# johncai117/Meta-Fine-Tuning

Measured on AMD Instinct MI355X. Metric: episodes/sec at 5-way N-shot (ResNet10+GNN) per GPU and 1/2/4/8-GPU node, higher is better.
Workload: dtype f32

## Files before the change

meta-fine-tuning_amd/csrc/conv_igemm.hip:

```cpp
#include "mft_common.h"
#include "mft_hip_testing.h"

int mft_stem_conv_dispatch(const float* in, const float* w, float* out, int n_img, int H, int W, int w_ld,
                           hipStream_t s);
int mft_skinny_fwd_dispatch(const float* in, int ldi, const float* w, float* out, int ldo, int n_img, int H, int W,
                            int Cin, int Cout, int KH, int KW, int stride, int pad, int imgs_per_group,
                            long long w_group_stride, hipStream_t s);
void mft_skinny_set_dgrad_slices(int n);
void mft_skinny_set_tap(int v);
void mft_skinny_set_x3(int v);
void mft_skinny_set_nw(int v);
void mft_bn_small_set_rows(int rows);
void mft_bn_fwd_small_set_rows(int rows);
void mft_skinny_set_lines(int v);
int mft_skinny_dgrad_dispatch(const float* dy, int ldy, const float* w, float* dx, int ldx, int n_img, int H, int W,
                              int Cin, int Cout, int KH, int KW, int stride, int pad, int imgs_per_group,
                              long long w_group_stride, hipStream_t s);

namespace {

struct ConvArgs {
    const float* in;
    const float* w;
    const float* bias;
    float* out;
    int ldi, ldo;
    int H, W, Cin, OH, OW, Cout, KH, KW, stride, pad;
    int Kpad;
    int Ktot;
    int rows_per_group;
    int imgs_per_group;
    int tiles_n;
    long long wgs;
    int bt_stride;
    int ksplit;
    float* ws;
    int parity;
};

constexpr int BK = 32;
constexpr int LDS_LD = 36;
int g_dgrad_parity = 1;
int g_wgrad_tile = 64;
int g_conv_tile = 0;
int g_wgrad_pol = 7;
int g_wgrad_trim = 1;
int g_wgrad_rows = 1;
int g_wgrad_early = 1;
int g_wgrad_min_lds_kb = 0;
int g_skinny = 1;
int g_stem_fast = 1;

template <int BM, int BN, int WM, int WN, bool STEM, bool BT>
__global__ __launch_bounds__(256) void conv_igemm_kernel(ConvArgs p) {
    constexpr int TM = BM / WM / 32;
    constexpr int TN = BN / WN / 32;
    constexpr int PA = BM / 32;
    constexpr int PB = BN / 32;
    extern __shared__ __attribute__((aligned(16))) float smem[];

    const int tid = threadIdx.x;
    const int lane = tid & 63;
    const int wave = tid >> 6;
    const int wm = wave / WN, wn = wave % WN;
    const int r = lane & 31, h = lane >> 5;

    int tile_id = blockIdx.x;
    if (gridDim.y == 1) {
        const int nwg = gridDim.x, q = nwg >> 3, rmd = nwg & 7;
        const int xcd = tile_id & 7, slot = tile_id >> 3;
        tile_id = xcd * q + (xcd < rmd ? xcd : rmd) + slot;
    }
    const int nt = tile_id % p.tiles_n;
    const int mt = tile_id / p.tiles_n;
    const bool par = BT && p.parity != 0;
    const int g = par ? 0 : blockIdx.y;
    const int ph = par ? (int)(blockIdx.y >> 1) : 0, pw = par ? (int)(blockIdx.y & 1) : 0;
    const int Hc = par ? (p.OH - ph + 1) / 2 : p.OH, Wc = par ? (p.OW - pw + 1) / 2 : p.OW;
    const int rows = par ? p.imgs_per_group * Hc * Wc : p.rows_per_group;
    const int m0 = mt * BM, n0 = nt * BN;
    if (par && m0 >= rows) return;
    const int kh0 = par ? ((ph - p.pad) & 1) : 0, kw0 = par ? ((pw - p.pad) & 1) : 0;
    const int nkh = par ? (p.KH - kh0 + 1) / 2 : p.KH, nkw = par ? (p.KW - kw0 + 1) / 2 : p.KW;

    const int lrow = tid >> 3;
    const int c4 = (tid & 7) * 4;
    const int ohw = Hc * Wc;

    long long a_base[PA];
    int a_ih0[PA], a_iw0[PA];
    bool a_ok[PA];
#pragma unroll
    for (int j = 0; j < PA; ++j) {
        int m = m0 + lrow + 32 * j;
        a_ok[j] = m < rows;
        int mm = a_ok[j] ? m : 0;
        int img = mm / ohw;
// ... 1041 lines not shown
    a.wgs = (groups > 1) ? w_group_stride : 0;
    a.tiles_n = 0;
    a.bt_stride = 1;
    a.ksplit = 1; a.ws = nullptr; a.parity = 0;
    if (ws != nullptr && !stem && ldo % 4 == 0) {
        a.ksplit = conv_ksplit(a.rows_per_group, Cout, a.Kpad, groups);
        a.ws = ws;
    }
    hipStream_t s = (hipStream_t)stream;
    if (stem) {
        if (g_stem_fast && KH == 7 && KW == 7 && stride == 2 && pad == 3 && Cout == 64 && ldi == 3 && ldo == 64 &&
            bias == nullptr && (W == 84 || W == 224)) {
            const int rc = mft_stem_conv_dispatch(in, w, out, n_img, H, W, a.Kpad, s);
            if (rc != MFT_EINVAL) return rc;
        }
        return launch_conv<128, 64, 2, 2, true>(a, groups, s);
    }
    if (g_skinny && groups > 1 && w_group_stride != 0 && bias == nullptr && ws == nullptr) {
        const int rc = mft_skinny_fwd_dispatch(in, ldi, w, out, ldo, n_img, H, W, Cin, Cout, KH, KW, stride, pad,
                                               imgs_per_group, w_group_stride, s);
        if (rc != MFT_EINVAL) return rc;
    }
    int tile = g_conv_tile;
    if (tile == 0) tile = (Cout >= 64) ? 4 : 5;
    switch (tile) {
        case 1: return launch_conv<128, 128, 2, 2, false>(a, groups, s);
        case 2: return launch_conv<128, 64, 2, 2, false>(a, groups, s);
        case 3: return launch_conv<64, 128, 2, 2, false>(a, groups, s);
        case 4: return launch_conv<64, 64, 2, 2, false>(a, groups, s);
        default: return launch_conv<128, 32, 4, 1, false>(a, groups, s);
    }
}

extern "C" int mft_conv2d_nhwc(const float* in, int ldi, const float* w, const float* bias, float* out, int ldo,
                               int n_img, int H, int W, int Cin, int Cout, int KH, int KW, int stride, int pad,
                               int imgs_per_group, long long w_group_stride, void* stream) {
    return conv2d_impl(in, ldi, w, bias, out, ldo, n_img, H, W, Cin, Cout, KH, KW, stride, pad, imgs_per_group, w_group_stride,
                       nullptr, stream);
}

extern "C" long long mft_conv_ksplit_ws_floats(long long rows, int cols, int K) {
    const int s = conv_ksplit(rows, cols, K);
    return s > 1 ? (long long)s * rows * cols : 0;
}

extern "C" long long mft_conv_ksplit_grouped_ws_floats(long long rows_per_group, int cols, int K, int groups) {
    const int s = conv_ksplit(rows_per_group, cols, K, groups);
    return s > 1 ? (long long)s * groups * rows_per_group * cols : 0;
}

extern "C" int mft_conv2d_nhwc_ksplit_grouped(const float* in, int ldi, const float* w, float* out, int ldo, int n_img, int H, int W,
                                              int Cin, int Cout, int KH, int KW, int stride, int pad, int imgs_per_group,
                                              long long w_group_stride, float* ws, void* stream) {
    if (ws == nullptr || imgs_per_group <= 0) return MFT_EINVAL;
    return conv2d_impl(in, ldi, w, nullptr, out, ldo, n_img, H, W, Cin, Cout, KH, KW, stride, pad, imgs_per_group, w_group_stride, ws,
                       stream);
}

extern "C" int mft_conv2d_nhwc_ksplit(const float* in, int ldi, const float* w, const float* bias, float* out, int ldo,
                                      int n_img, int H, int W, int Cin, int Cout, int KH, int KW, int stride, int pad, float* ws,
                                      void* stream) {
    return conv2d_impl(in, ldi, w, bias, out, ldo, n_img, H, W, Cin, Cout, KH, KW, stride, pad, 0, 0, ws, stream);
}

extern "C" int mft_has_experiments(void) {
#ifdef MFT_EXPERIMENTS
    return 1;
#else
    return 0;
#endif
}

extern "C" int mft_debug_set_conv_tile(int tile) {
#ifndef MFT_EXPERIMENTS
    if (tile == 9502 || tile == 9504 || tile == 9505) return MFT_EINVAL;
    if (tile >= 9000 && tile < 9100 && tile != 9003 && tile != 9007) return MFT_EINVAL;
    if (tile > 4000 && tile < 5000) return MFT_EINVAL;
#endif
    if (tile >= 11000) { mft_bn_small_set_rows(tile - 11000); mft_bn_fwd_small_set_rows(tile - 11000); }
    else if (tile >= 9800) g_dgrad_parity = tile - 9800;
    else if (tile >= 9700) mft_skinny_set_lines(tile - 9700);
    else if (tile >= 9600) g_wgrad_trim = tile - 9600;
    else if (tile >= 9500) g_wgrad_rows = tile - 9500;
    else if (tile >= 9100) mft_skinny_set_nw(tile - 9100);
    else if (tile >= 9000) g_wgrad_pol = tile - 9000;
    else if (tile >= 8000) mft_skinny_set_x3(tile - 8000);
    else if (tile >= 7000) mft_skinny_set_tap(tile - 7000);
    else if (tile >= 6000) mft_skinny_set_dgrad_slices(tile - 6000);
    else if (tile >= 5000) g_wgrad_early = tile - 5000;
    else if (tile >= 4000) g_wgrad_min_lds_kb = tile - 4000;
    else if (tile >= 3000) g_skinny = tile - 3000;
    else if (tile >= 2100) g_stem_wgrad_strips = tile - 2100;
    else if (tile >= 2000) g_stem_fast = tile - 2000;
    else if (tile >= 1000) g_wgrad_tile = tile - 1000;
    else g_conv_tile = tile;
    return 0;
}

extern "C" int mft_debug_set_x3_tile(int t);

extern "C" void mft_wgrad_fwd_set_exact(int on);
extern "C" int mft_debug_reset(void) {
    mft_wgrad_fwd_set_exact(0);
    mft_wgrad_fwd_set_xcd(1);
    g_dgrad_parity = 1; g_wgrad_trim = 1; g_wgrad_rows = 1; g_wgrad_tile = 64; g_conv_tile = 0; g_wgrad_pol = 7; g_wgrad_early = 1; g_wgrad_min_lds_kb = 0; g_skinny = 1; g_stem_fast = 1; g_stem_wgrad_strips = 1;
    mft_skinny_set_lines(1); mft_skinny_set_nw(0); mft_skinny_set_x3(1); mft_skinny_set_tap(1); mft_skinny_set_dgrad_slices(1);
    mft_debug_set_x3_tile(0); mft_debug_set_x3_tile(10); mft_debug_set_x3_tile(21); mft_debug_set_x3_tile(31); mft_debug_set_x3_tile(41);
    mft_bn_small_set_rows(512); mft_bn_fwd_small_set_rows(512);
    mft_debug_set_x3_tile(60); mft_debug_set_x3_tile(70); mft_debug_set_x3_tile(80); mft_debug_set_x3_tile(91); mft_debug_set_x3_tile(100); mft_debug_set_x3_tile(200);
    return 0;
}

static int dgrad_impl(const float* dy, int ldy, const float* w, float* dx, int ldx, int n_img, int H,
                      int W, int Cin, int Cout, int KH, int KW, int stride, int pad,
                      int imgs_per_group, long long w_group_stride, float* ws, void* stream) {
    if (Cout % 32 != 0 || Cin % 4 != 0 || ldy % 4 != 0 || stride < 1) return MFT_EINVAL;
    if (imgs_per_group <= 0) imgs_per_group = n_img;
    if (n_img % imgs_per_group != 0) return MFT_EINVAL;
    const int groups = n_img / imgs_per_group;
    if (g_skinny && groups > 1 && w_group_stride != 0 && ws == nullptr) {
        const int rc = mft_skinny_dgrad_dispatch(dy, ldy, w, dx, ldx, n_img, H, W, Cin, Cout, KH, KW, stride, pad,
                                                 imgs_per_group, w_group_stride, (hipStream_t)stream);
        if (rc != MFT_EINVAL) return rc;
    }
    ConvArgs a;
    a.in = dy; a.w = w; a.bias = nullptr; a.out = dx;
    a.ldi = ldy; a.ldo = ldx;
    a.H = (H + 2 * pad - KH) / stride + 1;
    a.W = (W + 2 * pad - KW) / stride + 1;
    a.Cin = Cout; a.KH = KH; a.KW = KW;
    a.stride = 1; a.pad = -pad;
    a.bt_stride = stride;
    a.OH = H; a.OW = W;
    a.Cout = Cin;
    a.Ktot = KH * KW * Cout;
    a.Kpad = a.Ktot;
    a.imgs_per_group = imgs_per_group;
    a.rows_per_group = imgs_per_group * H * W;
    a.wgs = (groups > 1) ? w_group_stride : 0;
    a.tiles_n = 0;
    a.ksplit = 1; a.ws = nullptr;
    a.parity = (groups == 1 && stride == 2 && g_dgrad_parity) ? 1 : 0;
    if (ws != nullptr && ldx % 4 == 0 && Cin % 64 == 0) {
        const int s_full = conv_ksplit(a.rows_per_group, Cin, a.Kpad, groups);
        if (!a.parity) {
            a.ksplit = s_full;
            a.ws = ws;
        } else if (s_full > 1) {
            int sp = conv_ksplit((long long)imgs_per_group * ((H + 1) / 2) * ((W + 1) / 2), Cin, ((KH + 1) / 2) * ((KW + 1) / 2) * Cout, 4);
            if (sp > s_full) sp = s_full;
            if (sp > 1) { a.ksplit = sp; a.ws = ws; }
        }
    }
    hipStream_t s = (hipStream_t)stream;
    if (Cin % 64 == 0) return launch_conv<64, 64, 2, 2, false, true>(a, groups, s);
    return launch_conv<128, 32, 4, 1, false, true>(a, groups, s);
}

extern "C" int mft_conv2d_dgrad_nhwc(const float* dy, int ldy, const float* w, float* dx, int ldx, int n_img, int H,
                                     int W, int Cin, int Cout, int KH, int KW, int stride, int pad,
                                     int imgs_per_group, long long w_group_stride, void* stream) {
    return dgrad_impl(dy, ldy, w, dx, ldx, n_img, H, W, Cin, Cout, KH, KW, stride, pad, imgs_per_group, w_group_stride, nullptr,
                      stream);
}

extern "C" int mft_conv2d_dgrad_nhwc_ksplit_grouped(const float* dy, int ldy, const float* w, float* dx, int ldx, int n_img, int H,
                                                    int W, int Cin, int Cout, int KH, int KW, int stride, int pad, int imgs_per_group,
                                                    long long w_group_stride, float* ws, void* stream) {
    if (ws == nullptr || imgs_per_group <= 0 || stride != 1) return MFT_EINVAL;
    return dgrad_impl(dy, ldy, w, dx, ldx, n_img, H, W, Cin, Cout, KH, KW, stride, pad, imgs_per_group, w_group_stride, ws, stream);
}

extern "C" int mft_conv2d_dgrad_nhwc_ksplit(const float* dy, int ldy, const float* w, float* dx, int ldx, int n_img, int H, int W,
                                            int Cin, int Cout, int KH, int KW, int stride, int pad, float* ws, void* stream) {
    return dgrad_impl(dy, ldy, w, dx, ldx, n_img, H, W, Cin, Cout, KH, KW, stride, pad, 0, 0, ws, stream);
}

extern "C" long long mft_conv2d_wgrad_ws_floats(int n_img, int H, int W, int Cin, int Cout, int KH, int KW, int stride,
                                                 int pad, int imgs_per_group) {
    if (imgs_per_group <= 0) imgs_per_group = n_img;
    const int OH = (H + 2 * pad - KH) / stride + 1, OW = (W + 2 * pad - KW) / stride + 1;
    const long long rows = (long long)imgs_per_group * OH * OW;
    int chunk_rows, chunks;
    wgrad_chunking(rows, wgrad_wgs_per_chunk(Cin, Cout, KH, KW, n_img / imgs_per_group), &chunk_rows, &chunks);
    if (chunks <= 1) return 0;
    const long long kpad = (KH * KW * Cin + 31) / 32 * 32;
    return (long long)(n_img / imgs_per_group) * chunks * Cout * kpad;
}

// ... 122 lines not shown
```

meta-fine-tuning_amd/csrc/skinny.hip:

```cpp
#include "mft_common.h"

namespace {

typedef float f32x4v __attribute__((ext_vector_type(4)));

struct SkinnyArgs {
    const float* act;
    const float* w;
    float* out;
    int lda, ldo;
    int H, W, Cin, OH, OW, Cout, KH, KW, stride, pad;
    int ipg, rows_in, rows_out;
    long long wgs;
    int K;
    int CS;
};

constexpr int SK_PADF = 8;
constexpr int SK_U = 8;

__global__ __launch_bounds__(1024) void skinny_conv_fwd_kernel(SkinnyArgs p) {
    extern __shared__ __attribute__((aligned(16))) float lds[];
    const int tid = threadIdx.x;
    const int lane = tid & 63, wave = tid >> 6;
// ... 718 lines not shown
    auto wptr = [&](int qq) { return qq < n_groups ? sk_wptr<LN>(wrow, qq, p.K) : sk_wptr<LN>(wsrow, qq - n_groups, p.Cin); };
    f32x4v a_cur[SK_U];
#pragma unroll
    for (int u = 0; u < SK_U; ++u) a_cur[u] = __builtin_nontemporal_load((const f32x4v*)sk_wptr<LN>(wrow, u, p.K));
    gather(0);
    scatter(0);
    __syncthreads();
    auto pass_body = [&](int pass, f32x4v (&A)[3]) {
        const unsigned short* L = ldh + (pass & 1) * 3 * PL + 8 * kq;
        for (int cg0 = 0; cg0 < gpt; cg0 += SK_U) {
            const int q0 = pass * gpt + cg0;
            const bool more = q0 + SK_U < n_groups + gpt;
#pragma unroll
            for (int u = 0; u < SK_U; u += 2) {
                bf16x8 a[3], b[3][3];
                sk_wfix<LN>(a_cur[u], a_cur[u + 1]);
                sk_split_a(a_cur[u], a_cur[u + 1], a);
                if (more) {
                    a_cur[u] = __builtin_nontemporal_load((const f32x4v*)wptr(q0 + SK_U + u));
                    a_cur[u + 1] = __builtin_nontemporal_load((const f32x4v*)wptr(q0 + SK_U + u + 1));
                }
#pragma unroll
                for (int nb = 0; nb < 3; ++nb)
#pragma unroll
                    for (int pl = 0; pl < 3; ++pl)
                        b[nb][pl] = __builtin_bit_cast(bf16x8, *(const u32x4v*)(L + pl * PL + (nb * 16 + m) * RS + (cg0 + u) * 16));
                SK_X3_MFMA(A, a, b)
            }
        }
    };
    for (int pass = 0; pass < taps; ++pass) {
        gather(pass + 1);
        pass_body(pass, acc);
        scatter((pass + 1) & 1);
        __syncthreads();
    }
    pass_body(taps, acs);

    const float inv = 1.f / (float)p.rows_out;
    f32x4v s = {0.f, 0.f, 0.f, 0.f};
#pragma unroll
    for (int nb = 0; nb < 3; ++nb)
        if (nb * 16 + m < p.rows_out) s += acc[nb];
    f32x4v mu, rs;
#pragma unroll
    for (int e = 0; e < 4; ++e) mu[e] = sk_row16_sum(s[e]) * inv;
    s = f32x4v{0.f, 0.f, 0.f, 0.f};
#pragma unroll
    for (int nb = 0; nb < 3; ++nb)
        if (nb * 16 + m < p.rows_out) {
            const f32x4v d = acc[nb] - mu;
            s += d * d;
        }
#pragma unroll
    for (int e = 0; e < 4; ++e) rs[e] = 1.0f / sqrtf(sk_row16_sum(s[e]) * inv + q.eps);
    const int co = co0 + 4 * kq;
    const f32x4v ga = *(const f32x4v*)(q.gamma + g * q.gbs + co), be = *(const f32x4v*)(q.beta + g * q.gbs + co);
    if (m == 0) {
        *(f32x4v*)(q.mean + (long long)g * p.Cout + co) = mu;
        *(f32x4v*)(q.rstd + (long long)g * p.Cout + co) = rs;
    }
    const long long ob = (long long)g * p.rows_out * p.ldo;
#pragma unroll
    for (int nb = 0; nb < 3; ++nb) {
        const int ro = nb * 16 + m;
        if (ro >= p.rows_out) continue;
        const long long o = ob + (long long)ro * p.ldo + co;
        *(f32x4v*)(p.out + o) = acc[nb];
        *(f32x4v*)(q.sc + o) = acs[nb];
        f32x4v y = (acc[nb] - mu) * rs * ga + be;
#pragma unroll
        for (int e = 0; e < 4; ++e) y[e] = fmaxf(y[e], 0.f);
        *(f32x4v*)(q.r1 + o) = y;
    }
}

struct SkinnyBnArgs {
    const float* x_raw;
    const float* relu_out;
    const float* mean; const float* rstd; const float* gamma; long long gbs;
    float* dgamma; float* dbeta;
};

template <bool BNB, int NW>
__global__ __launch_bounds__(64 * NW) void skinny_conv_dgrad_x3_kernel(SkinnyArgs p, SkinnyBnArgs bn) {
    extern __shared__ __attribute__((aligned(16))) unsigned short ldh[];
    typedef float f32x2v __attribute__((ext_vector_type(2)));
    const int tid = threadIdx.x;
    const int lane = tid & 63, wave = tid >> 6;
    const int m = lane & 15, kq = lane >> 4;
    const int g = blockIdx.y;
    const int ci0 = blockIdx.x * (32 * NW) + wave * 32;
    const int Cdy = p.Cin, Cdx = p.Cout;
    const int RS = Cdy + SK_PADH;
    const int PL = p.rows_in * RS;
    const int hw = p.H * p.W;
    const int taps = p.KH * p.KW;
    const long long co_stride = (long long)taps * Cdx;

    int n_img[3], n_h[3], n_w[3];
    bool n_ok[3];
#pragma unroll
    for (int nb = 0; nb < 3; ++nb) {
        const int ro = nb * 16 + m;
        n_ok[nb] = ro < p.rows_out;
        const int rr = n_ok[nb] ? ro : 0;
        const int img = rr / hw;
        const int rem = rr - img * hw;
        n_img[nb] = img;
        n_h[nb] = rem / p.W;
        n_w[nb] = rem - n_h[nb] * p.W;
    }
    const float* wbase = p.w + (long long)g * p.wgs + ci0 + 2 * m;
    const float* actg = p.act + (long long)g * p.rows_in * p.lda;

    constexpr int U = 4;
    const int gpt = Cdy / 16;
    const int n_groups = taps * gpt;
    f32x2v a_cur[U][4];
    auto load_group = [&](int q, f32x2v* dst) {
        const int tap = q / gpt;
        const int cg = q - tap * gpt;
#pragma unroll
        for (int t = 0; t < 4; ++t) {
            const int co = cg * 16 + 4 * kq + t;
            dst[t] = __builtin_nontemporal_load((const f32x2v*)(wbase + (long long)co * co_stride + (long long)tap * Cdx));
        }
    };
#pragma unroll
    for (int u = 0; u < U; ++u) load_group(u, a_cur[u]);
    {
        const int q4 = Cdy / 4;
        for (int i = tid; i < p.rows_in * q4; i += 64 * NW) {
            const int r = i / q4, c = (i - r * q4) * 4;
            sk_store3(ldh, r * RS + sk_perm(c), PL, *(const f32x4v*)(actg + (long long)r * p.lda + c));
        }
    }
    __syncthreads();

    f32x4v acc[2][3];
#pragma unroll
    for (int b = 0; b < 2; ++b)
#pragma unroll
        for (int nb = 0; nb < 3; ++nb) acc[b][nb] = f32x4v{0.f, 0.f, 0.f, 0.f};

    for (int q0 = 0; q0 < n_groups; q0 += U) {
        const bool more = q0 + U < n_groups;
        const int tap = q0 / gpt;
        const int cg0 = q0 - tap * gpt;
        const int kh = tap / p.KW, kw = tap - kh * p.KW;
        int boff[3];
#pragma unroll
        for (int nb = 0; nb < 3; ++nb) {
            const int ih = n_h[nb] + p.pad - kh, iw = n_w[nb] + p.pad - kw;
            const bool ok = n_ok[nb] && ih >= 0 && ih < p.H && iw >= 0 && iw < p.W;
            boff[nb] = ok ? ((n_img[nb] * p.H + ih) * p.W + iw) * RS + 8 * kq + cg0 * 16 : -1;
        }
#pragma unroll
        for (int u = 0; u < U; u += 2) {
            bf16x8 a[2][3], b[3][3];
#pragma unroll
            for (int bb = 0; bb < 2; ++bb) {
                const f32x4v w0 = {a_cur[u][0][bb], a_cur[u][1][bb], a_cur[u][2][bb], a_cur[u][3][bb]};
                const f32x4v w1 = {a_cur[u + 1][0][bb], a_cur[u + 1][1][bb], a_cur[u + 1][2][bb], a_cur[u + 1][3][bb]};
                sk_split_a(w0, w1, a[bb]);
            }
            if (more) {
                load_group(q0 + U + u, a_cur[u]);
                load_group(q0 + U + u + 1, a_cur[u + 1]);
            }
#pragma unroll
            for (int nb = 0; nb < 3; ++nb)
#pragma unroll
                for (int pl = 0; pl < 3; ++pl) {
                    u32x4v z = {0u, 0u, 0u, 0u};
                    if (boff[nb] >= 0) z = *(const u32x4v*)(ldh + pl * PL + boff[nb] + u * 16);
                    b[nb][pl] = __builtin_bit_cast(bf16x8, z);
                }
            SK_X3_MFMA(acc[0], a[0], b)
            SK_X3_MFMA(acc[1], a[1], b)
        }
    }
    float* outg = p.out + (long long)g * p.rows_out * p.ldo;
    f32x4v d[3][2];
#pragma unroll
    for (int nb = 0; nb < 3; ++nb) {
        d[nb][0][0] = acc[0][nb][0]; d[nb][0][1] = acc[1][nb][0]; d[nb][0][2] = acc[0][nb][1]; d[nb][0][3] = acc[1][nb][1];
        d[nb][1][0] = acc[0][nb][2]; d[nb][1][1] = acc[1][nb][2]; d[nb][1][2] = acc[0][nb][3]; d[nb][1][3] = acc[1][nb][3];
    }
    const int cc = ci0 + 8 * kq;
    if constexpr (BNB) {
        const long long gb = (long long)g * p.rows_out * p.ldo;
        f32x4v mu[2], rs[2], ga[2], xh[3][2], s1[2], s2[2];
#pragma unroll
        for (int h = 0; h < 2; ++h) {
            mu[h] = *(const f32x4v*)(bn.mean + (long long)g * Cdx + cc + 4 * h);
            rs[h] = *(const f32x4v*)(bn.rstd + (long long)g * Cdx + cc + 4 * h);
            ga[h] = *(const f32x4v*)(bn.gamma + g * bn.gbs + cc + 4 * h);
            s1[h] = s2[h] = f32x4v{0.f, 0.f, 0.f, 0.f};
        }
#pragma unroll
        for (int nb = 0; nb < 3; ++nb) {
            const int ro = nb * 16 + m;
#pragma unroll
            for (int h = 0; h < 2; ++h) {
                xh[nb][h] = f32x4v{0.f, 0.f, 0.f, 0.f};
                if (ro < p.rows_out) {
                    const long long o = gb + (long long)ro * p.ldo + cc + 4 * h;
                    const f32x4v r = *(const f32x4v*)(bn.relu_out + o);
                    xh[nb][h] = (*(const f32x4v*)(bn.x_raw + o) - mu[h]) * rs[h];
#pragma unroll
                    for (int e = 0; e < 4; ++e) d[nb][h][e] = r[e] > 0.f ? d[nb][h][e] : 0.f;
                    s1[h] += d[nb][h];
                    s2[h] += d[nb][h] * xh[nb][h];
                } else {
                    d[nb][h] = f32x4v{0.f, 0.f, 0.f, 0.f};
                }
            }
        }
        const float inv = 1.f / (float)p.rows_out;
#pragma unroll
        for (int h = 0; h < 2; ++h) {
#pragma unroll
            for (int e = 0; e < 4; ++e) {
                s1[h][e] = sk_row16_sum(s1[h][e]);
                s2[h][e] = sk_row16_sum(s2[h][e]);
            }
            if (m == 0) {
                *(f32x4v*)(bn.dgamma + (long long)g * Cdx + cc + 4 * h) = s2[h];
                *(f32x4v*)(bn.dbeta + (long long)g * Cdx + cc + 4 * h) = s1[h];
            }
            const f32x4v m1 = s1[h] * inv, m2 = s2[h] * inv, kk = ga[h] * rs[h];
#pragma unroll
            for (int nb = 0; nb < 3; ++nb) d[nb][h] = kk * (d[nb][h] - m1 - xh[nb][h] * m2);
        }
    }
#pragma unroll
    for (int nb = 0; nb < 3; ++nb) {
        const int ro = nb * 16 + m;
        if (ro >= p.rows_out) continue;
        float* o = outg + (long long)ro * p.ldo + cc;
        *(f32x4v*)(o) = d[nb][0];
        *(f32x4v*)(o + 4) = d[nb][1];
    }
}

int g_skinny_x3 = 1;
int g_skinny_tap = 1;
int g_skinny_dgrad_slices = 1;

int g_skinny_lines = 1;
int g_skinny_nw = 0;

inline int pick_nw(int groups, int wgs_per_group_at_max, int nw_max) {
    if (g_skinny_nw == 0) return nw_max;
    if (g_skinny_nw != 99) return g_skinny_nw <= nw_max ? (g_skinny_nw >= nw_max / 4 ? g_skinny_nw : nw_max / 4) : nw_max;
    int nw = nw_max;
    while (nw > nw_max / 4 && (long long)groups * wgs_per_group_at_max * (nw_max / nw) < 256) nw >>= 1;
    return nw;
}

template <typename K, typename... A>
int launch_big_lds(K kern, size_t max_lds, dim3 grid, dim3 block, size_t lds, hipStream_t s, A... args) {
    static std::mutex mu;
    static const void* done[256];
    static int done_dev[256];
    static int n_done = 0;
    int dev = 0;
    (void)hipGetDevice(&dev);
    bool seen = false;
    {
        std::lock_guard<std::mutex> lock(mu);
        for (int i = 0; i < n_done; ++i) seen = seen || (done[i] == (const void*)kern && done_dev[i] == dev);
    }
    if (!seen) {
        hipError_t e = hipFuncSetAttribute((const void*)kern, hipFuncAttributeMaxDynamicSharedMemorySize, (int)max_lds);
        if (e != hipSuccess) return (int)e;
        std::lock_guard<std::mutex> lock(mu);
        bool dup = false;
        for (int i = 0; i < n_done; ++i) dup = dup || (done[i] == (const void*)kern && done_dev[i] == dev);
        if (!dup && n_done < 256) { done[n_done] = (const void*)kern; done_dev[n_done] = dev; ++n_done; }
    }
    hipLaunchKernelGGL(kern, grid, block, lds, s, args...);
    return mft_launch_status();
}

int pick_slice(int rows_in, int Cin) {
    for (int cs = Cin; cs >= 128; cs /= 2) {
        if (cs % 128 != 0 || Cin % cs != 0) continue;
        if ((long long)rows_in * (cs + SK_PADF) * 4 <= 100 * 1024) return cs;
    }
    return 0;
}

}

void mft_skinny_set_dgrad_slices(int n) { g_skinny_dgrad_slices = n; }
void mft_skinny_set_tap(int v) { g_skinny_tap = v; }
void mft_skinny_set_x3(int v) { g_skinny_x3 = v; }
void mft_skinny_set_nw(int v) { g_skinny_nw = v; }
void mft_skinny_set_lines(int v) { g_skinny_lines = v; }

static int skinny_fwd_impl(const float* in, int ldi, const float* w, float* out, int ldo, int n_img, int H, int W,
                           int Cin, int Cout, int KH, int KW, int stride, int pad, int imgs_per_group,
                           long long w_group_stride, const SkinnyExitArgs* ex, hipStream_t s) {
    if (imgs_per_group <= 0 || w_group_stride == 0 || n_img % imgs_per_group != 0) return MFT_EINVAL;
    const int OH = (H + 2 * pad - KH) / stride + 1, OW = (W + 2 * pad - KW) / stride + 1;
    const int rows_out = imgs_per_group * OH * OW, rows_in = imgs_per_group * H * W;
    if (rows_out > 48 || Cout % 256 != 0 || Cin % 128 != 0 || ldi % 4 != 0 || ldo % 4 != 0) return MFT_EINVAL;
    const int cs = pick_slice(rows_in, Cin);
    SkinnyArgs p;
    p.act = in; p.w = w; p.out = out; p.lda = ldi; p.ldo = ldo;
    p.H = H; p.W = W; p.Cin = Cin; p.OH = OH; p.OW = OW; p.Cout = Cout; p.KH = KH; p.KW = KW; p.stride = stride; p.pad = pad;
    p.ipg = imgs_per_group; p.rows_in = rows_in; p.rows_out = rows_out; p.wgs = w_group_stride;
    p.K = KH * KW * Cin; p.CS = cs;
    dim3 grid(Cout / 256, n_img / imgs_per_group, 1);
    if (cs != Cin) {
        if (ex != nullptr) return MFT_EINVAL;
        if (Cin > 256 || Cin % (16 * SK_U) != 0 || g_skinny_tap == 0) return MFT_EINVAL;
        if (g_skinny_x3) {
            const size_t lds_h = (size_t)2 * 3 * 48 * (Cin + SK_PADH) * 2;
            static bool attr_tx = false;
            if (!attr_tx) {
                hipError_t e = hipFuncSetAttribute((const void*)skinny_conv_fwd_tap_x3_kernel<true>,
                                                   hipFuncAttributeMaxDynamicSharedMemorySize, 156 * 1024);
                if (e == hipSuccess)
                    e = hipFuncSetAttribute((const void*)skinny_conv_fwd_tap_x3_kernel<false>,
                                            hipFuncAttributeMaxDynamicSharedMemorySize, 156 * 1024);
                if (e != hipSuccess) return (int)e;
                attr_tx = true;
            }
            if (g_skinny_lines) hipLaunchKernelGGL(skinny_conv_fwd_tap_x3_kernel<true>, grid, dim3(1024), lds_h, s, p);
            else hipLaunchKernelGGL(skinny_conv_fwd_tap_x3_kernel<false>, grid, dim3(1024), lds_h, s, p);
            return mft_launch_status();
        }
        const size_t lds_t = (size_t)2 * 48 * (Cin + SK_PADF) * sizeof(float);
        static bool attr_t = false;
        if (!attr_t) {
            hipError_t e = hipFuncSetAttribute((const void*)skinny_conv_fwd_tap_kernel,
                                               hipFuncAttributeMaxDynamicSharedMemorySize, 110 * 1024);
            if (e != hipSuccess) return (int)e;
            attr_t = true;
        }
        hipLaunchKernelGGL(skinny_conv_fwd_tap_kernel, grid, dim3(1024), lds_t, s, p);
        return mft_launch_status();
    }
    if (g_skinny_x3 && (size_t)3 * rows_in * (Cin + SK_PADH) * 2 <= 150 * 1024 && Cin % (16 * SK_U) == 0) {
        size_t lds3 = (size_t)3 * rows_in * (Cin + SK_PADH) * 2;
        if (ex != nullptr && lds3 < (size_t)16 * 48 * 16 * 4) lds3 = (size_t)16 * 48 * 16 * 4;
        const int groups = n_img / imgs_per_group;
        const int nw = pick_nw(groups, Cout / 256, 16);
        const dim3 g2(Cout / (16 * nw), groups, 1);
        const SkinnyExitArgs e0 = ex ? *ex : SkinnyExitArgs{};
#define SK_FWD(EX, NW) (g_skinny_lines ? launch_big_lds(skinny_conv_fwd_x3_kernel<EX, NW, true>, 150 * 1024, g2, dim3(64 * NW), lds3, s, p, e0) \
                                       : launch_big_lds(skinny_conv_fwd_x3_kernel<EX, NW, false>, 150 * 1024, g2, dim3(64 * NW), lds3, s, p, e0))
        if (ex != nullptr) return nw == 16 ? SK_FWD(true, 16) : nw == 8 ? SK_FWD(true, 8) : SK_FWD(true, 4);
        return nw == 16 ? SK_FWD(false, 16) : nw == 8 ? SK_FWD(false, 8) : SK_FWD(false, 4);
#undef SK_FWD
    }
    if (ex != nullptr) return MFT_EINVAL;
    const size_t lds = (size_t)rows_in * (cs + SK_PADF) * sizeof(float);
    static MftPerDeviceOnce attr_once;
    if (attr_once.need()) {
        hipError_t e = hipFuncSetAttribute((const void*)skinny_conv_fwd_kernel, hipFuncAttributeMaxDynamicSharedMemorySize,
                                           110 * 1024);
        if (e != hipSuccess) return (int)e;
        attr_once.mark();
    }
    hipLaunchKernelGGL(skinny_conv_fwd_kernel, grid, dim3(1024), lds, s, p);
    return mft_launch_status();
}

static int skinny_dgrad_impl(const float* dy, int ldy, const float* w, float* dx, int ldx, int n_img, int H, int W,
                             int Cin, int Cout, int KH, int KW, int stride, int pad, int imgs_per_group,
                             long long w_group_stride, const SkinnyBnArgs* bn, hipStream_t s) {
    if (imgs_per_group <= 0 || w_group_stride == 0 || n_img % imgs_per_group != 0 || stride != 1) return MFT_EINVAL;
    if (2 * pad != KH - 1 || 2 * pad != KW - 1) return MFT_EINVAL;
    const int rows = imgs_per_group * H * W;
    if (rows > 48 || Cin % 256 != 0 || Cout % 64 != 0 || ldy % 4 != 0 || ldx % 4 != 0) return MFT_EINVAL;
    int cs = Cout;
    if (g_skinny_dgrad_slices > 1 && Cout % (64 * g_skinny_dgrad_slices) == 0) cs = Cout / g_skinny_dgrad_slices;
    if ((long long)rows * (cs + SK_PADF) * 4 > 100 * 1024) return MFT_EINVAL;
    SkinnyArgs p;
    p.act = dy; p.w = w; p.out = dx; p.lda = ldy; p.ldo = ldx;
    p.H = H; p.W = W; p.Cin = Cout; p.OH = H; p.OW = W; p.Cout = Cin; p.KH = KH; p.KW = KW; p.stride = 1; p.pad = pad;
    p.ipg = imgs_per_group; p.rows_in = rows; p.rows_out = rows; p.wgs = w_group_stride;
    p.K = KH * KW * Cin; p.CS = cs;
    dim3 grid(Cin / 256, n_img / imgs_per_group, 1);
    if (g_skinny_x3 && g_skinny_dgrad_slices <= 1 && (size_t)3 * rows * (Cout + SK_PADH) * 2 <= 150 * 1024 && Cout % 64 == 0) {
        const size_t lds3 = (size_t)3 * rows * (Cout + SK_PADH) * 2;
        const int groups = n_img / imgs_per_group;
        int nw = pick_nw(groups, Cin / 256, 8);
        if (nw > 8) nw = 8;
        const dim3 g2(Cin / (32 * nw), groups, 1);
        const SkinnyBnArgs b0 = bn ? *bn : SkinnyBnArgs{};
#define SK_DG(BB, NW) launch_big_lds(skinny_conv_dgrad_x3_kernel<BB, NW>, 150 * 1024, g2, dim3(64 * NW), lds3, s, p, b0)
        if (bn != nullptr) return nw == 8 ? SK_DG(true, 8) : nw == 4 ? SK_DG(true, 4) : SK_DG(true, 2);
        return nw == 8 ? SK_DG(false, 8) : nw == 4 ? SK_DG(false, 4) : SK_DG(false, 2);
#undef SK_DG
    }
    if (bn != nullptr) return MFT_EINVAL;
    const size_t lds = (size_t)rows * (cs + SK_PADF) * sizeof(float);
    static MftPerDeviceOnce attr_once;
    if (attr_once.need()) {
        hipError_t e = hipFuncSetAttribute((const void*)skinny_conv_dgrad_kernel, hipFuncAttributeMaxDynamicSharedMemorySize,
                                           110 * 1024);
        if (e != hipSuccess) return (int)e;
        attr_once.mark();
    }
    hipLaunchKernelGGL(skinny_conv_dgrad_kernel, grid, dim3(512), lds, s, p);
    return mft_launch_status();
}

int mft_skinny_fwd_dispatch(const float* in, int ldi, const float* w, float* out, int ldo, int n_img, int H, int W,
                            int Cin, int Cout, int KH, int KW, int stride, int pad, int imgs_per_group,
                            long long w_group_stride, hipStream_t s) {
    return skinny_fwd_impl(in, ldi, w, out, ldo, n_img, H, W, Cin, Cout, KH, KW, stride, pad, imgs_per_group, w_group_stride,
                           nullptr, s);
}

extern "C" int mft_block_exit_small_forward(const float* r1, const float* w_c2, long long w_group_stride, const float* sc,
                                            float* c2, float* out, float* pooled, int n_img, int H, int W, int C,
                                            int imgs_per_group, const float* gamma2, const float* beta2, const float* gamma_sc,
                                            const float* beta_sc, long long gb_group_stride, float* mean2, float* rstd2,
                                            float* mean_sc, float* rstd_sc, float eps, void* stream) {
    if (!sc || !out || !pooled || imgs_per_group <= 0) return MFT_EINVAL;
    SkinnyExitArgs ex{sc, out, pooled, gamma2, beta2, gamma_sc, beta_sc, gb_group_stride, mean2, rstd2, mean_sc, rstd_sc, eps,
                      H * W};
    return skinny_fwd_impl(r1, C, w_c2, c2, C, n_img, H, W, C, C, 3, 3, 1, 1, imgs_per_group, w_group_stride, &ex,
                           (hipStream_t)stream);
}

int mft_skinny_dgrad_dispatch(const float* dy, int ldy, const float* w, float* dx, int ldx, int n_img, int H, int W,
                              int Cin, int Cout, int KH, int KW, int stride, int pad, int imgs_per_group,
                              long long w_group_stride, hipStream_t s) {
    return skinny_dgrad_impl(dy, ldy, w, dx, ldx, n_img, H, W, Cin, Cout, KH, KW, stride, pad, imgs_per_group, w_group_stride,
                             nullptr, s);
}

extern "C" int mft_conv2d_dgrad_bn_backward_small(const float* dy, int ldy, const float* w, float* dx, int ldx, int n_img, int H,
                                                  int W, int Cin, int Cout, int KH, int KW, int pad, int imgs_per_group,
                                                  long long w_group_stride, const float* x_raw, const float* relu_out,
                                                  const float* mean, const float* rstd, const float* gamma,
                                                  long long gb_group_stride, float* dgamma, float* dbeta, void* stream) {
    if (!x_raw || !relu_out || !mean || !rstd || !gamma || !dgamma || !dbeta || ldx != Cin) return MFT_EINVAL;
    SkinnyBnArgs bn{x_raw, relu_out, mean, rstd, gamma, gb_group_stride, dgamma, dbeta};
    return skinny_dgrad_impl(dy, ldy, w, dx, ldx, n_img, H, W, Cin, Cout, KH, KW, 1, pad, imgs_per_group, w_group_stride, &bn,
                             (hipStream_t)stream);
}

extern "C" int mft_block_entry_small_forward(const float* x, int ldx, const float* w_c1, long long w1_group_stride,
                                             const float* w_sc, long long wsc_group_stride, float* c1, float* r1, float* sc,
                                             int n_img, int H, int W, int Cin, int Cout, int stride, int imgs_per_group,
                                             const float* gamma1, const float* beta1, long long gb_group_stride, float* mean1,
                                             float* rstd1, float eps, void* stream) {
    if (imgs_per_group <= 0 || n_img % imgs_per_group != 0 || w1_group_stride == 0 || wsc_group_stride == 0) return MFT_EINVAL;
    const int OH = (H + 2 - 3) / stride + 1, OW = (W + 2 - 3) / stride + 1;
    if ((H - 1) / stride + 1 != OH || (W - 1) / stride + 1 != OW) return MFT_EINVAL;
    const int rows_out = imgs_per_group * OH * OW;
    if (!g_skinny_x3 || rows_out > 48 || Cout % 256 != 0 || Cin % (16 * SK_U) != 0 || Cin > 256 || ldx % 4 != 0) return MFT_EINVAL;
    SkinnyEntryArgs q;
    SkinnyArgs& p = q.c;
    p.act = x; p.w = w_c1; p.out = c1; p.lda = ldx; p.ldo = Cout;
    p.H = H; p.W = W; p.Cin = Cin; p.OH = OH; p.OW = OW; p.Cout = Cout; p.KH = 3; p.KW = 3; p.stride = stride; p.pad = 1;
    p.ipg = imgs_per_group; p.rows_in = imgs_per_group * H * W; p.rows_out = rows_out; p.wgs = w1_group_stride;
    p.K = 9 * Cin; p.CS = Cin;
    q.w_sc = w_sc; q.wscs = wsc_group_stride; q.sc = sc; q.r1 = r1; q.gamma = gamma1; q.beta = beta1; q.gbs = gb_group_stride;
    q.mean = mean1; q.rstd = rstd1; q.eps = eps;
    const size_t lds_h = (size_t)2 * 3 * 48 * (Cin + SK_PADH) * 2;
    const int groups = n_img / imgs_per_group;
    const int nw = pick_nw(groups, Cout / 256, 16);
    const dim3 g2(Cout / (16 * nw), groups, 1);
#define SK_EN(NW) (g_skinny_lines ? launch_big_lds(skinny_block_entry_x3_kernel<NW, true>, 156 * 1024, g2, dim3(64 * NW), lds_h, (hipStream_t)stream, q) \
                                  : launch_big_lds(skinny_block_entry_x3_kernel<NW, false>, 156 * 1024, g2, dim3(64 * NW), lds_h, (hipStream_t)stream, q))
    return nw == 16 ? SK_EN(16) : nw == 8 ? SK_EN(8) : SK_EN(4);
#undef SK_EN
}
```

Baseline: 90.38.

## Add wide 64-channel-per-wave dgrad x3 kernel with deeper weight prefetch

```diff
diff --git a/meta-fine-tuning_amd/csrc/conv_igemm.hip b/meta-fine-tuning_amd/csrc/conv_igemm.hip
--- a/meta-fine-tuning_amd/csrc/conv_igemm.hip
+++ b/meta-fine-tuning_amd/csrc/conv_igemm.hip
@@ -13,6 +13,7 @@
 void mft_bn_small_set_rows(int rows);
 void mft_bn_fwd_small_set_rows(int rows);
 void mft_skinny_set_lines(int v);
+int mft_skinny_set_dgrad_form(int v);
 int mft_skinny_dgrad_dispatch(const float* dy, int ldy, const float* w, float* dx, int ldx, int n_img, int H, int W,
                               int Cin, int Cout, int KH, int KW, int stride, int pad, int imgs_per_group,
                               long long w_group_stride, hipStream_t s);
@@ -1220,6 +1221,7 @@
     else if (tile >= 9700) mft_skinny_set_lines(tile - 9700);
     else if (tile >= 9600) g_wgrad_trim = tile - 9600;
     else if (tile >= 9500) g_wgrad_rows = tile - 9500;
+    else if (tile >= 9200 && tile < 9300) return mft_skinny_set_dgrad_form(tile - 9200);
     else if (tile >= 9100) mft_skinny_set_nw(tile - 9100);
     else if (tile >= 9000) g_wgrad_pol = tile - 9000;
     else if (tile >= 8000) mft_skinny_set_x3(tile - 8000);
@@ -1242,7 +1244,7 @@
     mft_wgrad_fwd_set_exact(0);
     mft_wgrad_fwd_set_xcd(1);
     g_dgrad_parity = 1; g_wgrad_trim = 1; g_wgrad_rows = 1; g_wgrad_tile = 64; g_conv_tile = 0; g_wgrad_pol = 7; g_wgrad_early = 1; g_wgrad_min_lds_kb = 0; g_skinny = 1; g_stem_fast = 1; g_stem_wgrad_strips = 1;
-    mft_skinny_set_lines(1); mft_skinny_set_nw(0); mft_skinny_set_x3(1); mft_skinny_set_tap(1); mft_skinny_set_dgrad_slices(1);
+    mft_skinny_set_lines(1); mft_skinny_set_dgrad_form(20); mft_skinny_set_nw(0); mft_skinny_set_x3(1); mft_skinny_set_tap(1); mft_skinny_set_dgrad_slices(1);
     mft_debug_set_x3_tile(0); mft_debug_set_x3_tile(10); mft_debug_set_x3_tile(21); mft_debug_set_x3_tile(31); mft_debug_set_x3_tile(41);
     mft_bn_small_set_rows(512); mft_bn_fwd_small_set_rows(512);
     mft_debug_set_x3_tile(60); mft_debug_set_x3_tile(70); mft_debug_set_x3_tile(80); mft_debug_set_x3_tile(91); mft_debug_set_x3_tile(100); mft_debug_set_x3_tile(200);
diff --git a/meta-fine-tuning_amd/csrc/skinny.hip b/meta-fine-tuning_amd/csrc/skinny.hip
--- a/meta-fine-tuning_amd/csrc/skinny.hip
+++ b/meta-fine-tuning_amd/csrc/skinny.hip
@@ -824,7 +824,68 @@
     float* dgamma; float* dbeta;
 };
 
-template <bool BNB, int NW>
+template <bool BNB, int H>
+__device__ __forceinline__ void sk_dgrad_epilogue(const SkinnyArgs& p, const SkinnyBnArgs& bn, int g, int m, int cc,
+                                                  f32x4v (&d)[3][H]) {
+    const int Cdx = p.Cout;
+    if constexpr (BNB) {
+        const long long gb = (long long)g * p.rows_out * p.ldo;
+        f32x4v mu[H], rs[H], ga[H], xh[3][H], s1[H], s2[H];
+#pragma unroll
+        for (int h = 0; h < H; ++h) {
+            mu[h] = *(const f32x4v*)(bn.mean + (long long)g * Cdx + cc + 4 * h);
+            rs[h] = *(const f32x4v*)(bn.rstd + (long long)g * Cdx + cc + 4 * h);
+            ga[h] = *(const f32x4v*)(bn.gamma + g * bn.gbs + cc + 4 * h);
+            s1[h] = s2[h] = f32x4v{0.f, 0.f, 0.f, 0.f};
+        }
+#pragma unroll
+        for (int nb = 0; nb < 3; ++nb) {
+            const int ro = nb * 16 + m;
+#pragma unroll
+            for (int h = 0; h < H; ++h) {
+                xh[nb][h] = f32x4v{0.f, 0.f, 0.f, 0.f};
+                if (ro < p.rows_out) {
+                    const long long o = gb + (long long)ro * p.ldo + cc + 4 * h;
+                    const f32x4v r = *(const f32x4v*)(bn.relu_out + o);
+                    xh[nb][h] = (*(const f32x4v*)(bn.x_raw + o) - mu[h]) * rs[h];
+#pragma unroll
+                    for (int e = 0; e < 4; ++e) d[nb][h][e] = r[e] > 0.f ? d[nb][h][e] : 0.f;
+                    s1[h] += d[nb][h];
+                    s2[h] += d[nb][h] * xh[nb][h];
+                } else {
+                    d[nb][h] = f32x4v{0.f, 0.f, 0.f, 0.f};
+                }
+            }
+        }
+        const float inv = 1.f / (float)p.rows_out;
+#pragma unroll
+        for (int h = 0; h < H; ++h) {
+#pragma unroll
+            for (int e = 0; e < 4; ++e) {
+                s1[h][e] = sk_row16_sum(s1[h][e]);
+                s2[h][e] = sk_row16_sum(s2[h][e]);
+            }
+            if (m == 0) {
+                *(f32x4v*)(bn.dgamma + (long long)g * Cdx + cc + 4 * h) = s2[h];
+                *(f32x4v*)(bn.dbeta + (long long)g * Cdx + cc + 4 * h) = s1[h];
+            }
+            const f32x4v m1 = s1[h] * inv, m2 = s2[h] * inv, kk = ga[h] * rs[h];
+#pragma unroll
+            for (int nb = 0; nb < 3; ++nb) d[nb][h] = kk * (d[nb][h] - m1 - xh[nb][h] * m2);
+        }
+    }
+    float* outg = p.out + (long long)g * p.rows_out * p.ldo;
+#pragma unroll
+    for (int nb = 0; nb < 3; ++nb) {
+        const int ro = nb * 16 + m;
+        if (ro >= p.rows_out) continue;
+        float* o = outg + (long long)ro * p.ldo + cc;
+#pragma unroll
+        for (int h = 0; h < H; ++h) *(f32x4v*)(o + 4 * h) = d[nb][h];
+    }
+}
+
+template <bool BNB, int NW, int U>
 __global__ __launch_bounds__(64 * NW) void skinny_conv_dgrad_x3_kernel(SkinnyArgs p, SkinnyBnArgs bn) {
     extern __shared__ __attribute__((aligned(16))) unsigned short ldh[];
     typedef float f32x2v __attribute__((ext_vector_type(2)));
@@ -856,7 +917,6 @@
     const float* wbase = p.w + (long long)g * p.wgs + ci0 + 2 * m;
     const float* actg = p.act + (long long)g * p.rows_in * p.lda;
 
-    constexpr int U = 4;
     const int gpt = Cdy / 16;
     const int n_groups = taps * gpt;
     f32x2v a_cur[U][4];
@@ -923,68 +983,118 @@
             SK_X3_MFMA(acc[1], a[1], b)
         }
     }
-    float* outg = p.out + (long long)g * p.rows_out * p.ldo;
     f32x4v d[3][2];
 #pragma unroll
     for (int nb = 0; nb < 3; ++nb) {
         d[nb][0][0] = acc[0][nb][0]; d[nb][0][1] = acc[1][nb][0]; d[nb][0][2] = acc[0][nb][1]; d[nb][0][3] = acc[1][nb][1];
         d[nb][1][0] = acc[0][nb][2]; d[nb][1][1] = acc[1][nb][2]; d[nb][1][2] = acc[0][nb][3]; d[nb][1][3] = acc[1][nb][3];
     }
-    const int cc = ci0 + 8 * kq;
-    if constexpr (BNB) {
-        const long long gb = (long long)g * p.rows_out * p.ldo;
-        f32x4v mu[2], rs[2], ga[2], xh[3][2], s1[2], s2[2];
-#pragma unroll
-        for (int h = 0; h < 2; ++h) {
-            mu[h] = *(const f32x4v*)(bn.mean + (long long)g * Cdx + cc + 4 * h);
-            rs[h] = *(const f32x4v*)(bn.rstd + (long long)g * Cdx + cc + 4 * h);
-            ga[h] = *(const f32x4v*)(bn.gamma + g * bn.gbs + cc + 4 * h);
-            s1[h] = s2[h] = f32x4v{0.f, 0.f, 0.f, 0.f};
-        }
-#pragma unroll
-        for (int nb = 0; nb < 3; ++nb) {
-            const int ro = nb * 16 + m;
-#pragma unroll
-            for (int h = 0; h < 2; ++h) {
-                xh[nb][h] = f32x4v{0.f, 0.f, 0.f, 0.f};
-                if (ro < p.rows_out) {
-                    const long long o = gb + (long long)ro * p.ldo + cc + 4 * h;
-                    const f32x4v r = *(const f32x4v*)(bn.relu_out + o);
-                    xh[nb][h] = (*(const f32x4v*)(bn.x_raw + o) - mu[h]) * rs[h];
-#pragma unroll
-                    for (int e = 0; e < 4; ++e) d[nb][h][e] = r[e] > 0.f ? d[nb][h][e] : 0.f;
-                    s1[h] += d[nb][h];
-                    s2[h] += d[nb][h] * xh[nb][h];
-                } else {
-                    d[nb][h] = f32x4v{0.f, 0.f, 0.f, 0.f};
-                }
-            }
-        }
-        const float inv = 1.f / (float)p.rows_out;
-#pragma unroll
-        for (int h = 0; h < 2; ++h) {
-#pragma unroll
-            for (int e = 0; e < 4; ++e) {
-                s1[h][e] = sk_row16_sum(s1[h][e]);
-                s2[h][e] = sk_row16_sum(s2[h][e]);
-            }
-            if (m == 0) {
-                *(f32x4v*)(bn.dgamma + (long long)g * Cdx + cc + 4 * h) = s2[h];
-                *(f32x4v*)(bn.dbeta + (long long)g * Cdx + cc + 4 * h) = s1[h];
-            }
-            const f32x4v m1 = s1[h] * inv, m2 = s2[h] * inv, kk = ga[h] * rs[h];
-#pragma unroll
-            for (int nb = 0; nb < 3; ++nb) d[nb][h] = kk * (d[nb][h] - m1 - xh[nb][h] * m2);
-        }
-    }
+    sk_dgrad_epilogue<BNB, 2>(p, bn, g, m, ci0 + 8 * kq, d);
+}
+
+template <bool BNB, int NW, int U>
+__global__ __launch_bounds__(64 * NW) void skinny_conv_dgrad_x3_wide_kernel(SkinnyArgs p, SkinnyBnArgs bn) {
+    extern __shared__ __attribute__((aligned(16))) unsigned short ldh[];
+    const int tid = threadIdx.x;
+    const int lane = tid & 63, wave = tid >> 6;
+    const int m = lane & 15, kq = lane >> 4;
+    const int g = blockIdx.y;
+    const int ci0 = blockIdx.x * (64 * NW) + wave * 64;
+    const int Cdy = p.Cin, Cdx = p.Cout;
+    const int RS = Cdy + SK_PADH;
+    const int PL = p.rows_in * RS;
+    const int hw = p.H * p.W;
+    const int taps = p.KH * p.KW;
+    const long long co_stride = (long long)taps * Cdx;
+
+    int n_img[3], n_h[3], n_w[3];
+    bool n_ok[3];
 #pragma unroll
     for (int nb = 0; nb < 3; ++nb) {
         const int ro = nb * 16 + m;
-        if (ro >= p.rows_out) continue;
-        float* o = outg + (long long)ro * p.ldo + cc;
-        *(f32x4v*)(o) = d[nb][0];
-        *(f32x4v*)(o + 4) = d[nb][1];
-    }
+        n_ok[nb] = ro < p.rows_out;
+        const int rr = n_ok[nb] ? ro : 0;
+        const int img = rr / hw;
+        const int rem = rr - img * hw;
+        n_img[nb] = img;
+        n_h[nb] = rem / p.W;
+        n_w[nb] = rem - n_h[nb] * p.W;
+    }
+    const float* wbase = p.w + (long long)g * p.wgs + ci0 + 4 * m;
+    const float* actg = p.act + (long long)g * p.rows_in * p.lda;
+
+    const int gpt = Cdy / 16;
+    const int n_groups = taps * gpt;
+    f32x4v a_cur[U][4];
+    auto load_group = [&](int q, f32x4v* dst) {
+        const int tap = q / gpt;
+        const int cg = q - tap * gpt;
+#pragma unroll
+        for (int t = 0; t < 4; ++t) {
+            const int co = cg * 16 + 4 * kq + t;
+            dst[t] = __builtin_nontemporal_load((const f32x4v*)(wbase + (long long)co * co_stride + (long long)tap * Cdx));
+        }
+    };
+#pragma unroll
+    for (int u = 0; u < U; ++u) load_group(u, a_cur[u]);
+    {
+        const int q4 = Cdy / 4;
+        for (int i = tid; i < p.rows_in * q4; i += 64 * NW) {
+            const int r = i / q4, c = (i - r * q4) * 4;
+            sk_store3(ldh, r * RS + sk_perm(c), PL, *(const f32x4v*)(actg + (long long)r * p.lda + c));
+        }
+    }
+    __syncthreads();
+
+    f32x4v acc[4][3];
+#pragma unroll
+    for (int b = 0; b < 4; ++b)
+#pragma unroll
+        for (int nb = 0; nb < 3; ++nb) acc[b][nb] = f32x4v{0.f, 0.f, 0.f, 0.f};
+
+    for (int q0 = 0; q0 < n_groups; q0 += U) {
+        const bool more = q0 + U < n_groups;
+        const int tap = q0 / gpt;
+        const int cg0 = q0 - tap * gpt;
+        const int kh = tap / p.KW, kw = tap - kh * p.KW;
+        int boff[3];
+#pragma unroll
+        for (int nb = 0; nb < 3; ++nb) {
+            const int ih = n_h[nb] + p.pad - kh, iw = n_w[nb] + p.pad - kw;
+            const bool ok = n_ok[nb] && ih >= 0 && ih < p.H && iw >= 0 && iw < p.W;
+            boff[nb] = ok ? ((n_img[nb] * p.H + ih) * p.W + iw) * RS + 8 * kq + cg0 * 16 : -1;
+        }
+#pragma unroll
+        for (int u = 0; u < U; u += 2) {
+            bf16x8 a[4][3], b[3][3];
+#pragma unroll
+            for (int bb = 0; bb < 4; ++bb) {
+                const f32x4v w0 = {a_cur[u][0][bb], a_cur[u][1][bb], a_cur[u][2][bb], a_cur[u][3][bb]};
+                const f32x4v w1 = {a_cur[u + 1][0][bb], a_cur[u + 1][1][bb], a_cur[u + 1][2][bb], a_cur[u + 1][3][bb]};
+                sk_split_a(w0, w1, a[bb]);
+            }
+            if (more) {
+                load_group(q0 + U + u, a_cur[u]);
+                load_group(q0 + U + u + 1, a_cur[u + 1]);
+            }
+#pragma unroll
+            for (int nb = 0; nb < 3; ++nb)
+#pragma unroll
+                for (int pl = 0; pl < 3; ++pl) {
+                    u32x4v z = {0u, 0u, 0u, 0u};
+                    if (boff[nb] >= 0) z = *(const u32x4v*)(ldh + pl * PL + boff[nb] + u * 16);
+                    b[nb][pl] = __builtin_bit_cast(bf16x8, z);
+                }
+#pragma unroll
+            for (int bb = 0; bb < 4; ++bb) SK_X3_MFMA(acc[bb], a[bb], b)
+        }
+    }
+    f32x4v d[3][4];
+#pragma unroll
+    for (int nb = 0; nb < 3; ++nb)
+#pragma unroll
+        for (int e = 0; e < 4; ++e) d[nb][e] = f32x4v{acc[0][nb][e], acc[1][nb][e], acc[2][nb][e], acc[3][nb][e]};
+    sk_dgrad_epilogue<BNB, 4>(p, bn, g, m, ci0 + 16 * kq, d);
 }
 
 int g_skinny_x3 = 1;
@@ -992,6 +1102,9 @@
 int g_skinny_dgrad_slices = 1;
 
 int g_skinny_lines = 1;
+int g_skinny_dgrad_wide = 1;
+int g_skinny_dgrad_depth = 0;
+constexpr int SK_DG_WIDE_U = 8;
 int g_skinny_nw = 0;
 
 inline int pick_nw(int groups, int wgs_per_group_at_max, int nw_max) {
@@ -1042,6 +1155,13 @@
 void mft_skinny_set_x3(int v) { g_skinny_x3 = v; }
 void mft_skinny_set_nw(int v) { g_skinny_nw = v; }
 void mft_skinny_set_lines(int v) { g_skinny_lines = v; }
+int mft_skinny_set_dgrad_form(int v) {
+    const int wide = v / 20, depth = v % 20;
+    if (v < 0 || wide > 1 || (depth != 0 && depth != 4 && depth != 8 && depth != 16)) return MFT_EINVAL;
+    g_skinny_dgrad_wide = wide;
+    g_skinny_dgrad_depth = depth;
+    return 0;
+}
 
 static int skinny_fwd_impl(const float* in, int ldi, const float* w, float* out, int ldo, int n_img, int H, int W,
                            int Cin, int Cout, int KH, int KW, int stride, int pad, int imgs_per_group,
@@ -1136,9 +1256,21 @@
         if (nw > 8) nw = 8;
         const dim3 g2(Cin / (32 * nw), groups, 1);
         const SkinnyBnArgs b0 = bn ? *bn : SkinnyBnArgs{};
-#define SK_DG(BB, NW) launch_big_lds(skinny_conv_dgrad_x3_kernel<BB, NW>, 150 * 1024, g2, dim3(64 * NW), lds3, s, p, b0)
-        if (bn != nullptr) return nw == 8 ? SK_DG(true, 8) : nw == 4 ? SK_DG(true, 4) : SK_DG(true, 2);
-        return nw == 8 ? SK_DG(false, 8) : nw == 4 ? SK_DG(false, 4) : SK_DG(false, 2);
+        const bool wide = g_skinny_dgrad_wide && w_group_stride % 4 == 0 && ((uintptr_t)w & 15) == 0;
+        int U = g_skinny_dgrad_depth ? g_skinny_dgrad_depth : wide ? SK_DG_WIDE_U : 4;
+        while ((Cout / 16) % U != 0) U >>= 1;
+        if (nw != 8) U = 4;
+#define SK_DG(BB, NW, UU) launch_big_lds(skinny_conv_dgrad_x3_kernel<BB, NW, UU>, 150 * 1024, g2, dim3(64 * NW), lds3, s, p, b0)
+#define SK_DGW(BB, NW, UU) launch_big_lds(skinny_conv_dgrad_x3_wide_kernel<BB, NW, UU>, 150 * 1024, g2, dim3(64 * NW), lds3, s, p, b0)
+#define SK_DG_ALL(BB)                                                                                                        \
+    if (wide) return nw != 8 ? (nw == 4 ? SK_DGW(BB, 2, 4) : SK_DGW(BB, 1, 4))                                              \
+                             : U == 16 ? SK_DGW(BB, 4, 16) : U == 8 ? SK_DGW(BB, 4, 8) : SK_DGW(BB, 4, 4);                  \
+    return nw != 8 ? (nw == 4 ? SK_DG(BB, 4, 4) : SK_DG(BB, 2, 4))                                                          \
+                   : U == 16 ? SK_DG(BB, 8, 16) : U == 8 ? SK_DG(BB, 8, 8) : SK_DG(BB, 8, 4);
+        if (bn != nullptr) { SK_DG_ALL(true) }
+        SK_DG_ALL(false)
+#undef SK_DG_ALL
+#undef SK_DGW
 #undef SK_DG
     }
     if (bn != nullptr) return MFT_EINVAL;
```

Result: slower. 81.81 (-9.5%).
